# microsoft/OmniParser

Hardware: AMD Instinct MI355X
Metric: screenshots/sec end-to-end (detect+caption) @1920x1080 (higher is better)
Workload: dtype f32 (split-f16x3 MFMA)

## Files before the change

### omniparser_amd/csrc/gemm_dma.hip

```cpp
#include "omni_internal.h"
#include "gemm_common.h"
#include <string.h>
#include <type_traits>

OMNI_RANGE_GUARD_TU()

namespace {

typedef __attribute__((address_space(3))) void lds_void;

struct GemmArgs {
  const unsigned char* x; const unsigned char* w; const float* bias; const float* res; unsigned char* y;
  int M, N, K, nk;
  int ldi, in_coff, ldo, out_coff, ldr, res_coff;
  int mtiles, ntiles, xcd_order, xcd_n;
  float oscale;
};

template <int BM, int BN, int WM, int WN, int TM, int TN, int LDS_BYTES, int ACT, bool OSPLIT, bool RES>
__device__ __forceinline__ void gemm_epilogue(f32x16 (&acc)[TM][TN], const GemmArgs& a, unsigned char* lds, int m0, int n0, int wave, int lane) {
  constexpr int NW = WM * WN;
  const int wm = wave / WN, wn = wave % WN;
  const int hsel = lane >> 5;
  static_assert(TN % 2 == 0, "epilogue stages 64 channels (256 bytes per row) of a wave at a time");
  constexpr int EP = 272;
  static_assert(NW * 32 * EP <= LDS_BYTES, "epilogue staging must fit the LDS ring");
  __syncthreads();
  unsigned char* stg = lds + wave * (32 * EP);
  const float osc = a.oscale;
  float amax = 0.0f;
  const int rrow = lane >> 4, chunk = lane & 15;
  static_assert(!(RES && OSPLIT), "residual + format-B output is not a layer of this model");
#pragma unroll
  for (int jh = 0; jh < TN / 2; ++jh) {
    const int nw0 = n0 + wn * (BN / WN) + jh * 64;
    f32x4 bq[2][4];
#pragma unroll
    for (int j = 0; j < 2; ++j)
#pragma unroll
      for (int q = 0; q < 4; ++q)
        bq[j][q] = a.bias ? *reinterpret_cast<const f32x4*>(a.bias + nw0 + 4 * hsel + j * 32 + q * 8) : f32x4{0.f, 0.f, 0.f, 0.f};
    f32x4 rres[8];
    auto load_res = [&](int i) {
#pragma unroll
      for (int it = 0; it < 8; ++it) {
        const int m = min(m0 + wm * (BM / WM) + i * 32 + it * 4 + rrow, a.M - 1);
        rres[it] = *reinterpret_cast<const f32x4*>(a.res + (long long)m * a.ldr + a.res_coff + nw0 + chunk * 4);
      }
    };
    if constexpr (RES) load_res(0);
#pragma unroll
    for (int i = 0; i < TM; ++i) {
      unsigned char* wr = stg + (lane & 31) * EP;
#pragma unroll
      for (int j = 0; j < 2; ++j)
#pragma unroll
        for (int q = 0; q < 4; ++q) {
          const f32x16& ac = acc[i][jh * 2 + j];
          float v[4];
          if constexpr (ACT == OMNI_ACT_GELU) {
#pragma unroll
            for (int c = 0; c < 4; c += 2) {
              const f32x2 g = omni_gelu2(f32x2{ac[q * 4 + c], ac[q * 4 + c + 1]} * osc + f32x2{bq[j][q][c], bq[j][q][c + 1]});
              v[c] = g[0]; v[c + 1] = g[1];
            }
          } else {
#pragma unroll
            for (int c = 0; c < 4; ++c) {
              float t = ac[q * 4 + c] * osc + bq[j][q][c];
              if constexpr (ACT == OMNI_ACT_SILU) t = t / (1.0f + expf(-t));
              v[c] = t;
            }
          }
          const int cl = j * 32 + q * 8 + 4 * hsel;
          if constexpr (OSPLIT) {
            uint2 hi, lo;
            omni_split4(v, hi, lo, amax);
            *reinterpret_cast<uint2*>(wr + omni_split_off(cl)) = hi;
            *reinterpret_cast<uint2*>(wr + omni_split_off(cl) + 32) = lo;
          } else {
            *reinterpret_cast<f32x4*>(wr + cl * 4) = f32x4{v[0], v[1], v[2], v[3]};
          }
        }
      OMNI_WAVE_SYNC();
      const int mt0 = m0 + wm * (BM / WM) + i * 32;
      f32x4 ov[8];
#pragma unroll
      for (int it = 0; it < 8; ++it) {
        ov[it] = *reinterpret_cast<const f32x4*>(stg + (it * 4 + rrow) * EP + chunk * 16);
        if constexpr (RES) ov[it] += rres[it];
      }
      if constexpr (RES) { if (i + 1 < TM) load_res(i + 1); }
#pragma unroll
      for (int it = 0; it < 8; ++it) {
        const int m = mt0 + it * 4 + rrow;
        if (m < a.M) *reinterpret_cast<f32x4*>(a.y + ((long long)m * a.ldo + a.out_coff + nw0) * 4 + chunk * 16) = ov[it];
      }
      OMNI_WAVE_SYNC();
    }
  }
  if constexpr (OSPLIT) omni_report_range(amax);
}

template <int BM, int BN, int WM, int WN, int NSTAGE, int ACT, bool OSPLIT, bool RES, int SCHED = 0>
__global__ __launch_bounds__(WM * WN * 64, 2) void gemm_dma_kernel(GemmArgs a) {
#if defined(__HIP_DEVICE_COMPILE__)
  constexpr int NW = WM * WN;
  constexpr int TM = BM / (32 * WM), TN = BN / (32 * WN);
  constexpr int A_DMA = BM / (8 * NW), B_DMA = BN / (8 * NW);
  constexpr int DPS = A_DMA + B_DMA;
  constexpr int STAGE = (BM + BN) * 128;
  constexpr int NP = TM / 2;
  constexpr int NU = 2 * NP;
  constexpr int NM = 6 * TN;
  static_assert(TM % 2 == 0 && TN >= 1 && A_DMA >= 1 && B_DMA >= 1 && NSTAGE >= 2 && NSTAGE <= 4, "tile / wave grid mismatch");
  static_assert(BM * 128 + (TN - 1) * 4096 < 65536 && (TM - 1) * 4096 < 65536, "ds_read immediate offsets");
  __shared__ __attribute__((aligned(16))) unsigned char lds[NSTAGE * STAGE];

  const int tid = threadIdx.x, lane = tid & 63;
  const int wave = __builtin_amdgcn_readfirstlane(tid >> 6);
  const int wm = wave / WN, wn = wave % WN;
  int mt, nt;
  if (!tile_of_block(blockIdx.x, a.mtiles, a.ntiles, a.xcd_order, a.xcd_n, mt, nt)) return;
  const int m0 = __builtin_amdgcn_readfirstlane(mt) * BM, n0 = __builtin_amdgcn_readfirstlane(nt) * BN;

  const int rsub = lane >> 3, slot = lane & 7;
  unsigned voffA[A_DMA], voffB[B_DMA];
  auto pieceA = [&](int i) { return SCHED == 2 ? wave + NW * i : wave * A_DMA + i; };
#pragma unroll
  for (int i = 0; i < A_DMA; ++i) {
    const int rl = pieceA(i) * 8 + rsub;
    const int rr = min(rl, a.M - 1 - m0);
    voffA[i] = (unsigned)rr * (unsigned)(a.ldi * 4) + (unsigned)((slot ^ ((rl >> 1) & 7)) * 16);
  }
#pragma unroll
  for (int i = 0; i < B_DMA; ++i) {
    const int rl = (wave * B_DMA + i) * 8 + rsub;
    const int rr = min(rl, a.N - 1 - n0);
    voffB[i] = (unsigned)rr * (unsigned)(a.K * 4) + (unsigned)((slot ^ ((rl >> 1) & 7)) * 16);
  }
  const __amdgpu_buffer_rsrc_t rsrcA =
      __builtin_amdgcn_make_buffer_rsrc((void*)(a.x + ((long long)m0 * a.ldi + a.in_coff) * 4), 0, 0x7fffffff, 0x00020000);
  const __amdgpu_buffer_rsrc_t rsrcB =
      __builtin_amdgcn_make_buffer_rsrc((void*)(a.w + (long long)n0 * a.K * 4), 0, 0x7fffffff, 0x00020000);
  auto issue_piece = [&](int kt, int stage, int i) {
    const int so = kt * 128;
    if (i < A_DMA)
      __builtin_amdgcn_raw_ptr_buffer_load_lds(rsrcA, (lds_void*)(lds + stage * STAGE + pieceA(i) * 1024), 16, voffA[i], so, 0, 0);
    else
      __builtin_amdgcn_raw_ptr_buffer_load_lds(rsrcB, (lds_void*)(lds + stage * STAGE + BM * 128 + (wave * B_DMA + i - A_DMA) * 1024), 16,
                                               voffB[i - A_DMA], so, 0, 0);
  };
  auto issue = [&](int kt, int stage) {
#pragma unroll
    for (int i = 0; i < DPS; ++i) issue_piece(kt, stage, i);
  };

  const int swz = (lane >> 1) & 7, hsel = lane >> 5;
  int offA[4], offW[4];
#pragma unroll
  for (int gp = 0; gp < 4; ++gp) {
    const int c = ((((gp >> 1) * 4 + (gp & 1) * 2 + hsel) ^ swz)) * 16;
    offA[gp] = (wm * (BM / WM) + (lane & 31)) * 128 + c;
    offW[gp] = BM * 128 + (wn * (BN / WN) + (lane & 31)) * 128 + c;
  }
  struct AF { f16x8 h[2], l[2]; };
  struct WF { f16x8 h[TN], l[TN]; };
  auto loadA = [&](const unsigned char* st, int g, int ip, AF& f) {
#pragma unroll
    for (int t = 0; t < 2; ++t) {
      f.h[t] = *reinterpret_cast<const f16x8*>(st + offA[g * 2 + 0] + (ip * 2 + t) * 4096);
      f.l[t] = *reinterpret_cast<const f16x8*>(st + offA[g * 2 + 1] + (ip * 2 + t) * 4096);
    }
  };
  auto loadW = [&](const unsigned char* st, int g, WF& f) {
#pragma unroll
    for (int j = 0; j < TN; ++j) {
      f.h[j] = *reinterpret_cast<const f16x8*>(st + offW[g * 2 + 0] + j * 4096);
      f.l[j] = *reinterpret_cast<const f16x8*>(st + offW[g * 2 + 1] + j * 4096);
    }
  };

  f32x16 acc[TM][TN];
#pragma unroll
  for (int i = 0; i < TM; ++i)
#pragma unroll
    for (int j = 0; j < TN; ++j)
#pragma unroll
      for (int e = 0; e < 16; ++e) acc[i][j][e] = 0.0f;

  auto mma = [&](const AF& af, const WF& wf, int ip) {
#pragma unroll
    for (int t = 0; t < 2; ++t)
#pragma unroll
      for (int j = 0; j < TN; ++j)
        acc[ip * 2 + t][j] = __builtin_amdgcn_mfma_f32_32x32x16_f16(wf.h[j], af.h[t], acc[ip * 2 + t][j], 0, 0, 0);
#pragma unroll
    for (int t = 0; t < 2; ++t)
#pragma unroll
      for (int j = 0; j < TN; ++j)
        acc[ip * 2 + t][j] = __builtin_amdgcn_mfma_f32_32x32x16_f16(wf.l[j], af.h[t], acc[ip * 2 + t][j], 0, 0, 0);
#pragma unroll
    for (int t = 0; t < 2; ++t)
#pragma unroll
      for (int j = 0; j < TN; ++j)
        acc[ip * 2 + t][j] = __builtin_amdgcn_mfma_f32_32x32x16_f16(wf.h[j], af.l[t], acc[ip * 2 + t][j], 0, 0, 0);
  };

  const int nk = a.nk;
#pragma unroll
  for (int s = 0; s < NSTAGE - 1; ++s)
    if (s < nk) issue(s, s);
  int stage = 0, nstage = NSTAGE - 1;
  constexpr int IU = SCHED == 1 ? (NU + 1) / 2 : NU;
  constexpr int PPU = (DPS + IU - 1) / IU;
  AF af[2];
  WF wf[2];
  auto slice = [&](int kt, auto more_tag) {
    constexpr bool MORE = decltype(more_tag)::value;
    if constexpr (NSTAGE > 2 && MORE) OMNI_WAIT_VMCNT((NSTAGE - 2) * DPS);
    else OMNI_WAIT_VMCNT(0);
    __builtin_amdgcn_s_barrier();
    const unsigned char* st = lds + stage * STAGE;
    loadW(st, 0, wf[0]);
    loadA(st, 0, 0, af[0]);
#pragma unroll
    for (int u = 0; u < NU; ++u) {
      const int g = u / NP, ip = u % NP;
      int nds = 0;
      if (u + 1 < NU) {
        const int g2 = (u + 1) / NP, ip2 = (u + 1) % NP;
        if (g2 != g) { loadW(st, g2, wf[g2 & 1]); nds += 2 * TN; }
        loadA(st, g2, ip2, af[(u + 1) & 1]);
        nds += 4;
      }
      if constexpr (MORE) {
#pragma unroll
        for (int i = u * PPU; i < (u + 1) * PPU && i < DPS; ++i) issue_piece(kt + NSTAGE - 1, nstage, i);
      }
      mma(af[u & 1], wf[g & 1], ip);
      {
        const int npc = (MORE && u < IU) ? PPU : 0;
#pragma unroll
        for (int k = 0; k < NM; ++k) {
          __builtin_amdgcn_sched_group_barrier(0x8, 1, 0);
          if (k < nds) __builtin_amdgcn_sched_group_barrier(0x100, 1, 0);
          else if (k < nds + npc) __builtin_amdgcn_sched_group_barrier(0x20, 1, 0);
        }
      }
      __builtin_amdgcn_sched_barrier(0);
    }
    stage = stage + 1 == NSTAGE ? 0 : stage + 1;
    nstage = nstage + 1 == NSTAGE ? 0 : nstage + 1;
  };
  if constexpr (SCHED == 2) {
    static_assert(BM == 256 && BN == 256 && WM == 2 && WN == 4 && NSTAGE == 2 && TM == 4 && TN == 2 && A_DMA == 4 && B_DMA == 4, "ping-pong: 256x256 tile, 8 waves");
    OMNI_WAIT_VMCNT(0);
    __builtin_amdgcn_s_barrier();
    if (wm == 1) __builtin_amdgcn_s_barrier();
    auto phase_barrier = [&]() {
      __builtin_amdgcn_sched_barrier(0);
      __builtin_amdgcn_s_barrier();
      __builtin_amdgcn_sched_barrier(0);
    };
    {
      AF afp;
      auto slice_pp = [&](int kt, auto more_tag) {
        constexpr bool MORE = decltype(more_tag)::value;
        const unsigned char* st = lds + stage * STAGE;
#pragma unroll
        for (int u = 0; u < 4; ++u) {
          const int g = u & 1, ip = u >> 1;
          if (u < 2) loadW(st, g, wf[g]);
          loadA(st, g, ip, afp);
          if constexpr (MORE) {
            if (u == 0) { issue_piece(kt + 1, nstage, 0); issue_piece(kt + 1, nstage, 2); }
            if (u == 1) { issue_piece(kt + 1, nstage, A_DMA + 0); issue_piece(kt + 1, nstage, A_DMA + 1); }
            if (u == 2) { issue_piece(kt + 1, nstage, A_DMA + 2); issue_piece(kt + 1, nstage, A_DMA + 3); }
            if (u == 3) { issue_piece(kt + 1, nstage, 1); issue_piece(kt + 1, nstage, 3); }
            if (u == 1) OMNI_WAIT_VMCNT(4);
            if (u == 3) OMNI_WAIT_VMCNT(2);
          } else {
            if (u == 1) OMNI_WAIT_VMCNT(0);
          }
          phase_barrier();
          __builtin_amdgcn_s_setprio(1);
          mma(afp, wf[g], ip);
          __builtin_amdgcn_s_setprio(0);
          phase_barrier();
        }
        stage ^= 1;
        nstage ^= 1;
      };
      int ktp = 0;
      for (; ktp + 1 < nk; ++ktp) slice_pp(ktp, std::true_type{});
      for (; ktp < nk; ++ktp) slice_pp(ktp, std::false_type{});
    }
    if (wm == 0) __builtin_amdgcn_s_barrier();
  } else {
  int kt = 0;
  for (; kt + NSTAGE - 1 < nk; ++kt) slice(kt, std::true_type{});
  for (; kt < nk; ++kt) slice(kt, std::false_type{});
  }

  gemm_epilogue<BM, BN, WM, WN, TM, TN, NSTAGE * STAGE, ACT, OSPLIT, RES>(acc, a, lds, m0, n0, wave, lane);
#endif
}

__global__ __launch_bounds__(256) void split_convert_kernel(const float* __restrict__ x, unsigned char* __restrict__ y, long long rows,
                                                            int C, int ldi, int in_coff, int ldo, int out_coff) {
  const int gpr = C / 16;
  const long long idx = (long long)blockIdx.x * blockDim.x + threadIdx.x;
  if (idx >= rows * gpr) return;
  const long long r = idx / gpr;
  const int g = (int)(idx - r * gpr);
  const float* src = x + r * ldi + in_coff + g * 16;
  f32x4 v[4];
#pragma unroll
  for (int q = 0; q < 4; ++q) v[q] = *reinterpret_cast<const f32x4*>(src + q * 4);
  uint2 hi[4], lo[4];
#pragma unroll
  for (int q = 0; q < 4; ++q) {
    float t[4] = {v[q][0], v[q][1], v[q][2], v[q][3]};
    omni_split4(t, hi[q], lo[q]);
  }
  unsigned char* dst = y + (r * ldo + out_coff + g * 16) * 4;
  *reinterpret_cast<u32x4*>(dst) = u32x4{hi[0].x, hi[0].y, hi[1].x, hi[1].y};
  *reinterpret_cast<u32x4*>(dst + 16) = u32x4{hi[2].x, hi[2].y, hi[3].x, hi[3].y};
  *reinterpret_cast<u32x4*>(dst + 32) = u32x4{lo[0].x, lo[0].y, lo[1].x, lo[1].y};
  *reinterpret_cast<u32x4*>(dst + 48) = u32x4{lo[2].x, lo[2].y, lo[3].x, lo[3].y};
}

struct MlpArgs {
  const unsigned char* x; const unsigned char* w1; const unsigned char* w2; const float* b1;
  GemmArgs ep{};
  int ldi, in_coff;
  float osc1;
};

template <int C, int HID>
__global__ __launch_bounds__(256, 2) void mlp_fused_kernel(MlpArgs a) {
#if defined(__HIP_DEVICE_COMPILE__)
  static_assert(C == 128 && HID % 32 == 0, "written for the C = 128 stage: 8 K groups in registers, 4 output tiles");
  constexpr int NW = 4, KG = C / 16, OB = C / 32, NCH = HID / 32;
  constexpr int W1B = 32 * C * 4, W2B = C * 128, STAGE = W1B + W2B;
  constexpr int P1 = W1B / 1024 / NW, P2 = W2B / 1024 / NW;
  __shared__ __attribute__((aligned(16))) unsigned char lds[2 * STAGE + HID * 4];
  float* lb1 = reinterpret_cast<float*>(lds + 2 * STAGE);

  const int tid = threadIdx.x, lane = tid & 63;
  const int wave = __builtin_amdgcn_readfirstlane(tid >> 6);
  const int m0 = blockIdx.x * (NW * 32);
  const int hsel = lane >> 5, swz = (lane >> 1) & 7;

  for (int e = tid * 4; e < HID; e += 256 * 4) *reinterpret_cast<f32x4*>(lb1 + e) = *reinterpret_cast<const f32x4*>(a.b1 + e);

  const int rsub = lane >> 3, slot = lane & 7;
  unsigned voff1[P1], voff2[P2];
#pragma unroll
  for (int i = 0; i < P1; ++i) {
    const int pc = wave * P1 + i, rl = (pc & 3) * 8 + rsub, sl = pc >> 2;
    voff1[i] = (unsigned)rl * (unsigned)(C * 4) + (unsigned)(sl * 128) + (unsigned)((slot ^ ((rl >> 1) & 7)) * 16);
  }
#pragma unroll
  for (int i = 0; i < P2; ++i) {
    const int rl = (wave * P2 + i) * 8 + rsub;
    voff2[i] = (unsigned)rl * (unsigned)(HID * 4) + (unsigned)((slot ^ ((rl >> 1) & 7)) * 16);
  }
  const __amdgpu_buffer_rsrc_t rsrc1 = __builtin_amdgcn_make_buffer_rsrc((void*)a.w1, 0, 0x7fffffff, 0x00020000);
  const __amdgpu_buffer_rsrc_t rsrc2 = __builtin_amdgcn_make_buffer_rsrc((void*)a.w2, 0, 0x7fffffff, 0x00020000);
  auto issue = [&](int c, int stage) {
#pragma unroll
    for (int i = 0; i < P1; ++i)
      __builtin_amdgcn_raw_ptr_buffer_load_lds(rsrc1, (lds_void*)(lds + stage * STAGE + (wave * P1 + i) * 1024), 16, voff1[i], c * (32 * C * 4), 0, 0);
#pragma unroll
    for (int i = 0; i < P2; ++i)
      __builtin_amdgcn_raw_ptr_buffer_load_lds(rsrc2, (lds_void*)(lds + stage * STAGE + W1B + (wave * P2 + i) * 1024), 16, voff2[i], c * 128, 0, 0);
  };
  issue(0, 0);

  f16x8 xh[KG], xl[KG];
  {
    const int m = min(m0 + wave * 32 + (lane & 31), a.ep.M - 1);
    const unsigned char* xrow = a.x + ((long long)m * a.ldi + a.in_coff) * 4 + hsel * 16;
#pragma unroll
    for (int g = 0; g < KG; ++g) {
      xh[g] = *reinterpret_cast<const f16x8*>(xrow + g * 64);
      xl[g] = *reinterpret_cast<const f16x8*>(xrow + g * 64 + 32);
    }
  }
  int fo[2][2];
#pragma unroll
  for (int gg = 0; gg < 2; ++gg)
#pragma unroll
    for (int pt = 0; pt < 2; ++pt) fo[gg][pt] = (lane & 31) * 128 + (((gg * 4 + pt * 2 + hsel) ^ swz) * 16);

  f32x16 acc2[1][OB];
#pragma unroll
  for (int j = 0; j < OB; ++j)
#pragma unroll
    for (int e = 0; e < 16; ++e) acc2[0][j][e] = 0.0f;
  const float osc1 = a.osc1;
  float amax = 0.0f;
  __syncthreads();

  for (int c = 0; c < NCH; ++c) {
    const int stage = c & 1;
    OMNI_WAIT_VMCNT(0);
    __builtin_amdgcn_s_barrier();
    if (c + 1 < NCH) issue(c + 1, stage ^ 1);
    const unsigned char* st = lds + stage * STAGE;
    f32x16 a1[2];
#pragma unroll
    for (int e = 0; e < 16; ++e) { a1[0][e] = 0.0f; a1[1][e] = 0.0f; }
#pragma unroll
    for (int g = 0; g < KG; g += 2) {
      const unsigned char* sl = st + (g >> 1) * 4096;
      const f16x8 wh0 = *reinterpret_cast<const f16x8*>(sl + fo[0][0]), wl0 = *reinterpret_cast<const f16x8*>(sl + fo[0][1]);
      const f16x8 wh1 = *reinterpret_cast<const f16x8*>(sl + fo[1][0]), wl1 = *reinterpret_cast<const f16x8*>(sl + fo[1][1]);
      a1[0] = __builtin_amdgcn_mfma_f32_32x32x16_f16(wh0, xh[g], a1[0], 0, 0, 0);
      a1[1] = __builtin_amdgcn_mfma_f32_32x32x16_f16(wh1, xh[g + 1], a1[1], 0, 0, 0);
      a1[0] = __builtin_amdgcn_mfma_f32_32x32x16_f16(wl0, xh[g], a1[0], 0, 0, 0);
      a1[1] = __builtin_amdgcn_mfma_f32_32x32x16_f16(wl1, xh[g + 1], a1[1], 0, 0, 0);
      a1[0] = __builtin_amdgcn_mfma_f32_32x32x16_f16(wh0, xl[g], a1[0], 0, 0, 0);
      a1[1] = __builtin_amdgcn_mfma_f32_32x32x16_f16(wh1, xl[g + 1], a1[1], 0, 0, 0);
    }
    f16x8 gh[2], gl[2];
#pragma unroll
    for (int kg = 0; kg < 2; ++kg) {
      uint2 hq[2], lq[2];
#pragma unroll
      for (int qq = 0; qq < 2; ++qq) {
        const int q = kg * 2 + qq;
        const f32x4 bq = *reinterpret_cast<const f32x4*>(lb1 + c * 32 + 8 * q + 4 * hsel);
        float v[4];
#pragma unroll
        for (int r = 0; r < 4; r += 2) {
          const f32x2 t = omni_gelu2((f32x2{a1[0][q * 4 + r], a1[0][q * 4 + r + 1]} + f32x2{a1[1][q * 4 + r], a1[1][q * 4 + r + 1]}) * osc1 +
                                     f32x2{bq[r], bq[r + 1]});
          v[r] = t[0]; v[r + 1] = t[1];
        }
        omni_split4(v, hq[qq], lq[qq], amax);
      }
      gh[kg] = __builtin_bit_cast(f16x8, u32x4{hq[0].x, hq[0].y, hq[1].x, hq[1].y});
      gl[kg] = __builtin_bit_cast(f16x8, u32x4{lq[0].x, lq[0].y, lq[1].x, lq[1].y});
    }
#pragma unroll
    for (int kg = 0; kg < 2; ++kg)
#pragma unroll
      for (int j = 0; j < OB; j += 2) {
        const unsigned char* sw = st + W1B + j * 4096;
        const f16x8 wh0 = *reinterpret_cast<const f16x8*>(sw + fo[kg][0]), wl0 = *reinterpret_cast<const f16x8*>(sw + fo[kg][1]);
        const f16x8 wh1 = *reinterpret_cast<const f16x8*>(sw + 4096 + fo[kg][0]), wl1 = *reinterpret_cast<const f16x8*>(sw + 4096 + fo[kg][1]);
        acc2[0][j] = __builtin_amdgcn_mfma_f32_32x32x16_f16(wh0, gh[kg], acc2[0][j], 0, 0, 0);
        acc2[0][j + 1] = __builtin_amdgcn_mfma_f32_32x32x16_f16(wh1, gh[kg], acc2[0][j + 1], 0, 0, 0);
        acc2[0][j] = __builtin_amdgcn_mfma_f32_32x32x16_f16(wl0, gh[kg], acc2[0][j], 0, 0, 0);
        acc2[0][j + 1] = __builtin_amdgcn_mfma_f32_32x32x16_f16(wl1, gh[kg], acc2[0][j + 1], 0, 0, 0);
        acc2[0][j] = __builtin_amdgcn_mfma_f32_32x32x16_f16(wh0, gl[kg], acc2[0][j], 0, 0, 0);
        acc2[0][j + 1] = __builtin_amdgcn_mfma_f32_32x32x16_f16(wh1, gl[kg], acc2[0][j + 1], 0, 0, 0);
      }
  }
  omni_report_range(amax);
  gemm_epilogue<NW * 32, C, NW, 1, 1, OB, 2 * STAGE, OMNI_ACT_NONE, false, true>(acc2, a.ep, lds, m0, 0, wave, lane);
#endif
}

template <int BM, int BN, int WM, int WN, int NSTAGE>
int launch_tile(GemmArgs& a, int act, int osplit, hipStream_t s) {
  a.mtiles = (a.M + BM - 1) / BM;
  a.ntiles = a.N / BN;
  a.xcd_order = (a.mtiles >= 64 && a.ntiles > 1) ? 1 : 0;
  a.xcd_n = a.xcd_order ? choose_xcd_n(a.ntiles, 4ll * a.N * a.K) : 1;
  dim3 grid(tile_grid(a.mtiles, a.ntiles, a.xcd_order, a.xcd_n)), block(WM * WN * 64);
  const bool res = a.res != nullptr;
  constexpr int SCHED1 = (BM == 256 && BN == 256) ? 1 : 0;
  const char* sched_e = getenv("OMNI_GEMM_SCHED");
  const bool lockstep = sched_e && atoi(sched_e) == 1;
#define OMNI_GD(ACT_, OS_, RES_)                                                                                                   \
  do {                                                                                                                             \
    if constexpr (BM == 256 && BN == 256) {                                                                                        \
      if (!lockstep) { hipLaunchKernelGGL((gemm_dma_kernel<BM, BN, WM, WN, NSTAGE, ACT_, OS_, RES_, 2>), grid, block, 0, s, a); break; }  \
    }                                                                                                                              \
    hipLaunchKernelGGL((gemm_dma_kernel<BM, BN, WM, WN, NSTAGE, ACT_, OS_, RES_, SCHED1>), grid, block, 0, s, a);                  \
  } while (0)
  if (act == OMNI_ACT_NONE && !osplit && !res) OMNI_GD(OMNI_ACT_NONE, false, false);
  else if (act == OMNI_ACT_NONE && !osplit && res) OMNI_GD(OMNI_ACT_NONE, false, true);
  else if (act == OMNI_ACT_NONE && osplit && !res) OMNI_GD(OMNI_ACT_NONE, true, false);
  else if (act == OMNI_ACT_GELU && osplit && !res) OMNI_GD(OMNI_ACT_GELU, true, false);
  else if (act == OMNI_ACT_GELU && !osplit && !res) OMNI_GD(OMNI_ACT_GELU, false, false);
#undef OMNI_GD
  else {
    omni_set_error("gemm_dma: unsupported epilogue (act %d, split out %d, residual %d)", act, osplit, (int)res);
    return OMNI_E_ARG;
  }
  return OMNI_OK;
}

}

int omni_launch_gemm_dma(const omni_op_t* op, hipStream_t s) {
  GemmArgs a{};
  a.x = (const unsigned char*)op->p[0]; a.w = (const unsigned char*)op->p[1]; a.bias = (const float*)op->p[2];
  a.res = (const float*)op->p[3]; a.y = (unsigned char*)op->p[4];
  const int B = op->i[0], H = op->i[1], W = op->i[2];
  a.K = op->i[3]; a.ldi = op->i[4]; a.in_coff = op->i[5];
  a.N = op->i[12]; a.ldo = op->i[13]; a.out_coff = op->i[14];
  const int act = op->i[15];
  a.ldr = op->i[16]; a.res_coff = op->i[17];
  const int osplit = op->i[21];
  a.oscale = op->f[1] != 0.0f ? op->f[1] : 1.0f;
  OMNI_REQUIRE(op->dtype == OMNI_F32, "gemm_dma: f32 plans only");
  OMNI_REQUIRE(a.x && a.w && a.y, "gemm_dma: null pointer");
  OMNI_REQUIRE(op->i[6] == 1 && op->i[7] == 1 && op->i[8] == 1 && op->i[9] == 0 && op->i[10] == H && op->i[11] == W,
               "gemm_dma: pointwise layers only");
  OMNI_REQUIRE(op->f[0] == 0.0f, "gemm_dma: output scale is not supported");
  const long long M = (long long)B * H * W;
  OMNI_REQUIRE(M > 0 && M < (1ll << 31), "gemm_dma: bad M");
  a.M = (int)M;
  OMNI_REQUIRE(a.K >= 32 && a.K % 32 == 0 && a.N % 128 == 0, "gemm_dma: needs K %% 32 == 0 and N %% 128 == 0 (K %d, N %d)", a.K, a.N);
  OMNI_REQUIRE(a.ldi % 16 == 0 && a.in_coff % 16 == 0, "gemm_dma: split input needs 16-channel aligned ld / offset (%d, %d)", a.ldi, a.in_coff);
  OMNI_REQUIRE(a.ldo % 4 == 0 && a.out_coff % 4 == 0 && (!osplit || (a.ldo % 16 == 0 && a.out_coff % 16 == 0)), "gemm_dma: output alignment");
  OMNI_REQUIRE(!a.res || (a.ldr % 4 == 0 && a.res_coff % 4 == 0), "gemm_dma: residual alignment");
  OMNI_REQUIRE((long long)a.ldi * 4 * 256 < (1ll << 31) && (long long)a.K * 4 * 256 < (1ll << 31), "gemm_dma: row stride too large");
  a.nk = a.K / 32;
  int tile = (a.N % 256 == 0) ? 0 : 1;
  {
    const long long mt256 = (a.M + 255) / 256;
    if (mt256 * (a.N / (tile == 0 ? 256 : 128)) < 256) tile = (tile == 0 && mt256 * (a.N / 128) >= 256) ? 1 : 2;
  }
  if (const char* e = getenv("OMNI_GEMM_TILE")) {
    if (!strcmp(e, "256x128")) tile = 1;
    else if (!strcmp(e, "128x128")) tile = 2;
    else if (!strcmp(e, "256x256") && a.N % 256 == 0) tile = 0;
  }
  int rc;
  if (tile == 0) rc = launch_tile<256, 256, 2, 4, 2>(a, act, osplit, s);
  else if (tile == 1) rc = launch_tile<256, 128, 4, 2, 3>(a, act, osplit, s);
  else rc = launch_tile<128, 128, 2, 2, 2>(a, act, osplit, s);
  if (rc) return rc;
  OMNI_HIP_CHECK(hipGetLastError());
  return OMNI_OK;
}

int omni_launch_split_convert(const omni_op_t* op, hipStream_t s) {
  const long long rows = (long long)op->i[0] * (op->i[1] > 0 ? op->i[1] : 1);
  const int C = op->i[3], ldi = op->i[4], in_coff = op->i[5], ldo = op->i[13], out_coff = op->i[14];
  OMNI_REQUIRE(op->dtype == OMNI_F32 && op->p[0] && op->p[4], "split_convert: f32 plans, non-null pointers");
  OMNI_REQUIRE(rows > 0 && C > 0 && C % 16 == 0 && ldi % 16 == 0 && in_coff % 16 == 0 && ldo % 16 == 0 && out_coff % 16 == 0,
               "split_convert: 16-channel alignment (C %d, ld %d/%d, off %d/%d)", C, ldi, ldo, in_coff, out_coff);
  const long long total = rows * (C / 16);
  hipLaunchKernelGGL(split_convert_kernel, dim3((unsigned)((total + 255) / 256)), dim3(256), 0, s, (const float*)op->p[0],
                     (unsigned char*)op->p[4], rows, C, ldi, in_coff, ldo, out_coff);
  OMNI_HIP_CHECK(hipGetLastError());
  return OMNI_OK;
}

int omni_launch_mlp_fused(const omni_op_t* op, hipStream_t s) {
  MlpArgs a{};
  a.x = (const unsigned char*)op->p[0]; a.w1 = (const unsigned char*)op->p[1]; a.b1 = (const float*)op->p[2];
  a.w2 = (const unsigned char*)op->p[5];
  a.ep.x = nullptr; a.ep.w = nullptr; a.ep.bias = (const float*)op->p[6]; a.ep.res = (const float*)op->p[3]; a.ep.y = (unsigned char*)op->p[4];
  const long long M = (long long)op->i[0] * (op->i[1] > 0 ? op->i[1] : 1);
  const int C = op->i[3], HID = op->i[12];
  a.ldi = op->i[4]; a.in_coff = op->i[5];
  a.ep.ldo = op->i[13]; a.ep.out_coff = op->i[14]; a.ep.ldr = op->i[16]; a.ep.res_coff = op->i[17];
  a.osc1 = op->f[1] != 0.0f ? op->f[1] : 1.0f;
  a.ep.oscale = op->f[2] != 0.0f ? op->f[2] : 1.0f;
  OMNI_REQUIRE(op->dtype == OMNI_F32, "mlp_fused: f32 plans only");
  OMNI_REQUIRE(a.x && a.w1 && a.w2 && a.b1 && a.ep.bias && a.ep.res && a.ep.y, "mlp_fused: null pointer (both biases and the residual are required)");
  OMNI_REQUIRE(C == 128 && HID == 512, "mlp_fused: built for C = 128, hidden = 512 (got %d, %d)", C, HID);
  OMNI_REQUIRE(M > 0 && M < (1ll << 31), "mlp_fused: bad row count");
  OMNI_REQUIRE(a.ldi % 16 == 0 && a.in_coff % 16 == 0, "mlp_fused: split input needs 16-channel aligned ld / offset");
  OMNI_REQUIRE(a.ep.ldo % 4 == 0 && a.ep.out_coff % 4 == 0 && a.ep.ldr % 4 == 0 && a.ep.res_coff % 4 == 0, "mlp_fused: output / residual alignment");
  a.ep.M = (int)M; a.ep.N = C; a.ep.K = HID; a.ep.nk = 0; a.ep.ldi = 0; a.ep.in_coff = 0;
  a.ep.mtiles = a.ep.ntiles = a.ep.xcd_order = a.ep.xcd_n = 0;
  hipLaunchKernelGGL((mlp_fused_kernel<128, 512>), dim3((unsigned)((M + 127) / 128)), dim3(256), 0, s, a);
  OMNI_HIP_CHECK(hipGetLastError());
  return OMNI_OK;
}
```

Before: 12.60.

## Software-pipeline fused MLP: overlap next fc1 MFMAs with current GELU and fc2

Restructures the fused fc1-GELU-fc2 chunk loop so that fc1 for chunk c+1 runs while GELU/split of chunk c is computed and fc2 of chunk c is issued. W1 and W2 DMA loads are staggered (W1 prefetched two chunks ahead, W2 one ahead), and the loop is unrolled by two with explicit sched_group_barrier interleaving of MFMA, LDS reads and VALU work. The goal is to hide the GELU/split VALU latency and LDS read latency behind matrix-core work. In exchange it raises register pressure (two fc1 accumulator sets, double-buffered fragments) and relies on hard-coded shape asserts (KG==8, OB==4, even NCH).

```diff
diff --git a/omniparser_amd/csrc/gemm_dma.hip b/omniparser_amd/csrc/gemm_dma.hip
--- a/omniparser_amd/csrc/gemm_dma.hip
+++ b/omniparser_amd/csrc/gemm_dma.hip
@@ -369,15 +369,17 @@
   }
   const __amdgpu_buffer_rsrc_t rsrc1 = __builtin_amdgcn_make_buffer_rsrc((void*)a.w1, 0, 0x7fffffff, 0x00020000);
   const __amdgpu_buffer_rsrc_t rsrc2 = __builtin_amdgcn_make_buffer_rsrc((void*)a.w2, 0, 0x7fffffff, 0x00020000);
-  auto issue = [&](int c, int stage) {
+  auto issue1 = [&](int c) {
 #pragma unroll
     for (int i = 0; i < P1; ++i)
-      __builtin_amdgcn_raw_ptr_buffer_load_lds(rsrc1, (lds_void*)(lds + stage * STAGE + (wave * P1 + i) * 1024), 16, voff1[i], c * (32 * C * 4), 0, 0);
+      __builtin_amdgcn_raw_ptr_buffer_load_lds(rsrc1, (lds_void*)(lds + (c & 1) * STAGE + (wave * P1 + i) * 1024), 16, voff1[i], c * (32 * C * 4), 0, 0);
+  };
+  auto issue2 = [&](int c) {
 #pragma unroll
     for (int i = 0; i < P2; ++i)
-      __builtin_amdgcn_raw_ptr_buffer_load_lds(rsrc2, (lds_void*)(lds + stage * STAGE + W1B + (wave * P2 + i) * 1024), 16, voff2[i], c * 128, 0, 0);
-  };
-  issue(0, 0);
+      __builtin_amdgcn_raw_ptr_buffer_load_lds(rsrc2, (lds_void*)(lds + (c & 1) * STAGE + W1B + (wave * P2 + i) * 1024), 16, voff2[i], c * 128, 0, 0);
+  };
+  issue1(0);
 
   f16x8 xh[KG], xl[KG];
   {
@@ -389,6 +391,8 @@
       xl[g] = *reinterpret_cast<const f16x8*>(xrow + g * 64 + 32);
     }
   }
+  issue1(1);
+  issue2(0);
   int fo[2][2];
 #pragma unroll
   for (int gg = 0; gg < 2; ++gg)
@@ -402,63 +406,121 @@
     for (int e = 0; e < 16; ++e) acc2[0][j][e] = 0.0f;
   const float osc1 = a.osc1;
   float amax = 0.0f;
+
+  struct WF { f16x8 f[4]; };
+  auto load1 = [&](const unsigned char* w1s, int u, WF& w) {
+    const unsigned char* sl = w1s + u * 4096;
+    w.f[0] = *reinterpret_cast<const f16x8*>(sl + fo[0][0]); w.f[1] = *reinterpret_cast<const f16x8*>(sl + fo[0][1]);
+    w.f[2] = *reinterpret_cast<const f16x8*>(sl + fo[1][0]); w.f[3] = *reinterpret_cast<const f16x8*>(sl + fo[1][1]);
+  };
+  auto mma1 = [&](int u, const WF& w, f32x16 (&a1)[2]) {
+    const int g = 2 * u;
+    a1[0] = __builtin_amdgcn_mfma_f32_32x32x16_f16(w.f[0], xh[g], a1[0], 0, 0, 0);
+    a1[1] = __builtin_amdgcn_mfma_f32_32x32x16_f16(w.f[2], xh[g + 1], a1[1], 0, 0, 0);
+    a1[0] = __builtin_amdgcn_mfma_f32_32x32x16_f16(w.f[1], xh[g], a1[0], 0, 0, 0);
+    a1[1] = __builtin_amdgcn_mfma_f32_32x32x16_f16(w.f[3], xh[g + 1], a1[1], 0, 0, 0);
+    a1[0] = __builtin_amdgcn_mfma_f32_32x32x16_f16(w.f[0], xl[g], a1[0], 0, 0, 0);
+    a1[1] = __builtin_amdgcn_mfma_f32_32x32x16_f16(w.f[2], xl[g + 1], a1[1], 0, 0, 0);
+  };
+  auto load2 = [&](const unsigned char* w2s, int u, WF& w) {
+    const int kg = u / (OB / 2), j = 2 * (u % (OB / 2));
+    const unsigned char* sw = w2s + j * 4096;
+    w.f[0] = *reinterpret_cast<const f16x8*>(sw + fo[kg][0]); w.f[1] = *reinterpret_cast<const f16x8*>(sw + fo[kg][1]);
+    w.f[2] = *reinterpret_cast<const f16x8*>(sw + 4096 + fo[kg][0]); w.f[3] = *reinterpret_cast<const f16x8*>(sw + 4096 + fo[kg][1]);
+  };
+  auto mma2 = [&](int u, const WF& w, const f16x8 (&gh)[2], const f16x8 (&gl)[2]) {
+    const int kg = u / (OB / 2), j = 2 * (u % (OB / 2));
+    acc2[0][j] = __builtin_amdgcn_mfma_f32_32x32x16_f16(w.f[0], gh[kg], acc2[0][j], 0, 0, 0);
+    acc2[0][j + 1] = __builtin_amdgcn_mfma_f32_32x32x16_f16(w.f[2], gh[kg], acc2[0][j + 1], 0, 0, 0);
+    acc2[0][j] = __builtin_amdgcn_mfma_f32_32x32x16_f16(w.f[1], gh[kg], acc2[0][j], 0, 0, 0);
+    acc2[0][j + 1] = __builtin_amdgcn_mfma_f32_32x32x16_f16(w.f[3], gh[kg], acc2[0][j + 1], 0, 0, 0);
+    acc2[0][j] = __builtin_amdgcn_mfma_f32_32x32x16_f16(w.f[0], gl[kg], acc2[0][j], 0, 0, 0);
+    acc2[0][j + 1] = __builtin_amdgcn_mfma_f32_32x32x16_f16(w.f[2], gl[kg], acc2[0][j + 1], 0, 0, 0);
+  };
+  struct GS { f32x4 bq[4]; float v[4]; uint2 hq[2], lq[2]; };
+  auto load_bias = [&](int c, int q, GS& s) { s.bq[q] = *reinterpret_cast<const f32x4*>(lb1 + c * 32 + 8 * q + 4 * hsel); };
+  auto gelu_piece = [&](const f32x16 (&a1)[2], int piece, GS& s, f16x8 (&gh)[2], f16x8 (&gl)[2]) {
+    const int q = piece / 3, h = piece % 3;
+    if (h < 2) {
+      const int r = 2 * h;
+      s.v[r] = omni_gelu((a1[0][q * 4 + r] + a1[1][q * 4 + r]) * osc1 + s.bq[q][r]);
+      s.v[r + 1] = omni_gelu((a1[0][q * 4 + r + 1] + a1[1][q * 4 + r + 1]) * osc1 + s.bq[q][r + 1]);
+    } else {
+      omni_split4(s.v, s.hq[q & 1], s.lq[q & 1], amax);
+      if (q & 1) {
+        gh[q >> 1] = __builtin_bit_cast(f16x8, u32x4{s.hq[0].x, s.hq[0].y, s.hq[1].x, s.hq[1].y});
+        gl[q >> 1] = __builtin_bit_cast(f16x8, u32x4{s.lq[0].x, s.lq[0].y, s.lq[1].x, s.lq[1].y});
+      }
+    }
+  };
+
+  static_assert(NCH % 2 == 0 && NCH >= 2 && KG == 8 && OB == 4, "the chunk loop is unrolled by two; four fc1 + four fc2 units per step");
+  constexpr int NU1 = KG / 2, NU = NU1 + OB;
+  constexpr int VPM = 14;
+  f32x16 a1[2][2];
+  f16x8 gh[2], gl[2];
+  WF wf[2];
+  GS gs;
+  auto zero1 = [&](f32x16 (&a)[2]) {
+#pragma unroll
+    for (int e = 0; e < 16; ++e) { a[0][e] = 0.0f; a[1][e] = 0.0f; }
+  };
+  OMNI_WAIT_VMCNT(P1 + P2);
   __syncthreads();
-
-  for (int c = 0; c < NCH; ++c) {
-    const int stage = c & 1;
+  zero1(a1[0]);
+#pragma unroll
+  for (int u = 0; u < NU1; ++u) {
+    load1(lds, u, wf[0]);
+    mma1(u, wf[0], a1[0]);
+  }
+  auto step = [&](int c, auto ptag) {
+    constexpr int P = decltype(ptag)::value;
     OMNI_WAIT_VMCNT(0);
     __builtin_amdgcn_s_barrier();
-    if (c + 1 < NCH) issue(c + 1, stage ^ 1);
-    const unsigned char* st = lds + stage * STAGE;
-    f32x16 a1[2];
-#pragma unroll
-    for (int e = 0; e < 16; ++e) { a1[0][e] = 0.0f; a1[1][e] = 0.0f; }
-#pragma unroll
-    for (int g = 0; g < KG; g += 2) {
-      const unsigned char* sl = st + (g >> 1) * 4096;
-      const f16x8 wh0 = *reinterpret_cast<const f16x8*>(sl + fo[0][0]), wl0 = *reinterpret_cast<const f16x8*>(sl + fo[0][1]);
-      const f16x8 wh1 = *reinterpret_cast<const f16x8*>(sl + fo[1][0]), wl1 = *reinterpret_cast<const f16x8*>(sl + fo[1][1]);
-      a1[0] = __builtin_amdgcn_mfma_f32_32x32x16_f16(wh0, xh[g], a1[0], 0, 0, 0);
-      a1[1] = __builtin_amdgcn_mfma_f32_32x32x16_f16(wh1, xh[g + 1], a1[1], 0, 0, 0);
-      a1[0] = __builtin_amdgcn_mfma_f32_32x32x16_f16(wl0, xh[g], a1[0], 0, 0, 0);
-      a1[1] = __builtin_amdgcn_mfma_f32_32x32x16_f16(wl1, xh[g + 1], a1[1], 0, 0, 0);
-      a1[0] = __builtin_amdgcn_mfma_f32_32x32x16_f16(wh0, xl[g], a1[0], 0, 0, 0);
-      a1[1] = __builtin_amdgcn_mfma_f32_32x32x16_f16(wh1, xl[g + 1], a1[1], 0, 0, 0);
-    }
-    f16x8 gh[2], gl[2];
-#pragma unroll
-    for (int kg = 0; kg < 2; ++kg) {
-      uint2 hq[2], lq[2];
-#pragma unroll
-      for (int qq = 0; qq < 2; ++qq) {
-        const int q = kg * 2 + qq;
-        const f32x4 bq = *reinterpret_cast<const f32x4*>(lb1 + c * 32 + 8 * q + 4 * hsel);
-        float v[4];
-#pragma unroll
-        for (int r = 0; r < 4; r += 2) {
-          const f32x2 t = omni_gelu2((f32x2{a1[0][q * 4 + r], a1[0][q * 4 + r + 1]} + f32x2{a1[1][q * 4 + r], a1[1][q * 4 + r + 1]}) * osc1 +
-                                     f32x2{bq[r], bq[r + 1]});
-          v[r] = t[0]; v[r + 1] = t[1];
-        }
-        omni_split4(v, hq[qq], lq[qq], amax);
-      }
-      gh[kg] = __builtin_bit_cast(f16x8, u32x4{hq[0].x, hq[0].y, hq[1].x, hq[1].y});
-      gl[kg] = __builtin_bit_cast(f16x8, u32x4{lq[0].x, lq[0].y, lq[1].x, lq[1].y});
-    }
-#pragma unroll
-    for (int kg = 0; kg < 2; ++kg)
-#pragma unroll
-      for (int j = 0; j < OB; j += 2) {
-        const unsigned char* sw = st + W1B + j * 4096;
-        const f16x8 wh0 = *reinterpret_cast<const f16x8*>(sw + fo[kg][0]), wl0 = *reinterpret_cast<const f16x8*>(sw + fo[kg][1]);
-        const f16x8 wh1 = *reinterpret_cast<const f16x8*>(sw + 4096 + fo[kg][0]), wl1 = *reinterpret_cast<const f16x8*>(sw + 4096 + fo[kg][1]);
-        acc2[0][j] = __builtin_amdgcn_mfma_f32_32x32x16_f16(wh0, gh[kg], acc2[0][j], 0, 0, 0);
-        acc2[0][j + 1] = __builtin_amdgcn_mfma_f32_32x32x16_f16(wh1, gh[kg], acc2[0][j + 1], 0, 0, 0);
-        acc2[0][j] = __builtin_amdgcn_mfma_f32_32x32x16_f16(wl0, gh[kg], acc2[0][j], 0, 0, 0);
-        acc2[0][j + 1] = __builtin_amdgcn_mfma_f32_32x32x16_f16(wl1, gh[kg], acc2[0][j + 1], 0, 0, 0);
-        acc2[0][j] = __builtin_amdgcn_mfma_f32_32x32x16_f16(wh0, gl[kg], acc2[0][j], 0, 0, 0);
-        acc2[0][j + 1] = __builtin_amdgcn_mfma_f32_32x32x16_f16(wh1, gl[kg], acc2[0][j + 1], 0, 0, 0);
-      }
+    if (c + 2 < NCH) issue1(c + 2);
+    issue2(c + 1);
+    const unsigned char* w1s = lds + (P ^ 1) * STAGE;
+    const unsigned char* w2s = lds + P * STAGE + W1B;
+    zero1(a1[P ^ 1]);
+    load1(w1s, 0, wf[0]);
+    load_bias(c, 0, gs);
+    __builtin_amdgcn_sched_barrier(0);
+#pragma unroll
+    for (int u = 0; u < NU; ++u) {
+      int nds = 0;
+      if (u + 1 < NU1) { load1(w1s, u + 1, wf[(u + 1) & 1]); nds += 4; }
+      else if (u + 1 < NU) { load2(w2s, u + 1 - NU1, wf[(u + 1) & 1]); nds += 4; }
+      if (u < 3) { load_bias(c, u + 1, gs); nds += 1; }
+      if (u < NU1) mma1(u, wf[u & 1], a1[P ^ 1]);
+      else mma2(u - NU1, wf[u & 1], gh, gl);
+      if (u < 6) {
+        gelu_piece(a1[P], 2 * u, gs, gh, gl);
+        gelu_piece(a1[P], 2 * u + 1, gs, gh, gl);
+      }
+#pragma unroll
+      for (int k = 0; k < 6; ++k) {
+        __builtin_amdgcn_sched_group_barrier(0x8, 1, 0);
+        if (k >= 6 - nds) __builtin_amdgcn_sched_group_barrier(0x100, 1, 0);
+        if (u < 6) __builtin_amdgcn_sched_group_barrier(0x2, VPM, 0);
+      }
+      if (u & 1) __builtin_amdgcn_sched_barrier(0);
+    }
+  };
+  for (int c = 0; c + 2 < NCH; c += 2) {
+    step(c, std::integral_constant<int, 0>{});
+    step(c + 1, std::integral_constant<int, 1>{});
+  }
+  step(NCH - 2, std::integral_constant<int, 0>{});
+  OMNI_WAIT_VMCNT(0);
+  __builtin_amdgcn_s_barrier();
+#pragma unroll
+  for (int q = 0; q < 4; ++q) load_bias(NCH - 1, q, gs);
+#pragma unroll
+  for (int piece = 0; piece < 12; ++piece) gelu_piece(a1[1], piece, gs, gh, gl);
+#pragma unroll
+  for (int u = 0; u < OB; ++u) {
+    load2(lds + STAGE + W1B, u, wf[0]);
+    mma2(u, wf[0], gh, gl);
   }
   omni_report_range(amax);
   gemm_epilogue<NW * 32, C, NW, 1, 1, OB, 2 * STAGE, OMNI_ACT_NONE, false, true>(acc2, a.ep, lds, m0, 0, wave, lane);
```

Result: no change. 12.65 (median of 4 runs) (+0.4%).
